# ufal/neuralmonkey

Measured on NVIDIA H100. Metric: train_target_tokens_per_sec, higher is better.
Workload: dtype f32 storage; tensor-core products in fp16 (vocabulary) / tf32 with fp32 accumulation

## Files before the change

include/nmb200.h:

```cpp
#ifndef NMB200_H
#define NMB200_H

#include <stdint.h>

#ifdef __cplusplus
extern "C" {
#endif

#define NM_ABI_VERSION 1

#define NM_OK 0
#define NM_E_INVALID (-1)
#define NM_E_UNSUPPORTED (-2)
#define NM_E_NO_DEVICE (-3)

#define NM_ACT_NONE 0
#define NM_ACT_TANH 1
#define NM_ACT_RELU 2
#define NM_ACT_SIGMOID 3

#define NM_GEMM_AUTO 0
#define NM_GEMM_SIMT 1
#define NM_GEMM_TC 2

// ... 98 lines not shown
int nm_xent_fwd(float* logits, int64_t unk_index, const int64_t* targets, const float* weights,
                float* lse, float* xent, int64_t* argmax, int64_t M, int64_t V,
                int64_t ldl, void* stream);
int nm_xent_bwd(const float* logits, const int64_t* targets, const float* weights,
                const float* lse, const float* scale, float* dlogits, int64_t M,
                int64_t V, int64_t ldl, void* stream);
int nm_log_softmax(const float* logits, const float* lse, float* logprobs,
                   int64_t M, int64_t V, int64_t ldl, void* stream);

int64_t nm_logits_xent_scratch(int64_t M, int64_t V);
int nm_logits_xent_fwd(const float* X, int64_t ldx, const float* W, int64_t ldw,
                       int transW, const float* b, int64_t unk_index, const int64_t* targets,
                       const float* weights, float* lse, float* xent,
                       int64_t* argmax, float* part, float* logits_out,
                       int64_t ldl, int64_t M, int64_t V, int64_t K, void* stream);
int nm_logits_xent_bwd(const float* X, int64_t ldx, const float* W, int64_t ldw,
                       int transW, const float* b, int64_t unk_index, const int64_t* targets,
                       const float* weights, const float* lse, const float* scale,
                       float* dlogits, int64_t ldd, int64_t M, int64_t V,
                       int64_t K, void* stream);

int nm_cast_f16(const float* src, int64_t ld_src, void* dst, int64_t ld_dst, int64_t rows,
                int64_t cols, const float* row_scale, int transpose, int extra_ones, void* stream);
int nm_gemm_f16(int64_t M, int64_t N, int64_t K, const void* A16, int64_t lda, const void* B16,
                int64_t ldb, float* C, int64_t ldc, const float* alpha_dev, const float* row_scale,
                float beta, int transposed, void* stream);
int nm_gemm_f16_tn(int64_t M, int64_t N, int64_t K, const void* A16, int64_t lda, const void* B16,
                   int64_t ldb, float* C, int64_t ldc, const float* alpha_dev, float beta, void* stream);
int nm_gemm_f16_tn_ctas(int64_t M, int64_t N, int64_t K, const void* A16, int64_t lda, const void* B16,
                        int64_t ldb, float* C, int64_t ldc, const float* alpha_dev, float beta, int max_ctas,
                        void* stream);
int nm_logits_xent_fwd16(const void* X16, int64_t ldx, const void* WT16, int64_t ldw, const float* b,
                         int64_t unk_index, const int64_t* targets, const float* weights, float* lse,
                         float* xent, int64_t* argmax, float* part, float* logits_out, int64_t ldl,
                         int64_t M, int64_t V, int64_t K, void* stream);
int nm_logits_xent_bwd16(const void* X16, int64_t ldx, const void* WT16, int64_t ldw, const float* b,
                         int64_t unk_index, const int64_t* targets, const float* mask, const float* lse,
                         void* dl16, int64_t ldd, int64_t M, int64_t V, int64_t K, void* stream);

int nm_beam_step(const float* logprobs, const float* logprob_sum,
                 const int32_t* lengths, const uint8_t* finished, float alpha,
                 float* scores, int64_t* word_ids, int32_t* beam_ids,
                 float* logprob_sum_out, int32_t* lengths_out,
                 uint8_t* finished_out, void* scratch, int64_t B, int64_t k,
                 int64_t V, void* stream);
int64_t nm_beam_scratch(int64_t B, int64_t k, int64_t V);
// ... 172 lines not shown
```

neuralmonkey_b200/build.py:

```python
import concurrent.futures
import os
import shutil
import subprocess
import sys
from typing import List

PKG_DIR = os.path.dirname(os.path.abspath(__file__))
CSRC = os.path.join(PKG_DIR, "csrc")
OBJ_DIR = os.path.join(PKG_DIR, "build")
LIB_PATH = os.path.join(PKG_DIR, "libnmb200.so")
HEADER = os.path.join(os.path.dirname(PKG_DIR), "include", "nmb200.h")

NVCC_FLAGS = [
    "-gencode", "arch=compute_90a,code=sm_90a",
    "-O3", "-lineinfo", "-std=c++17",
    "-Xcompiler", "-fPIC",
]


def _nvcc() -> str:
    nvcc = shutil.which("nvcc") or "/usr/local/cuda/bin/nvcc"
    if not os.path.exists(nvcc):
        raise RuntimeError("nvcc not found: cannot build libnmb200.so")
    return nvcc


def sources() -> List[str]:
    return sorted(f for f in os.listdir(CSRC) if f.endswith(".cu"))


def _deps_mtime() -> float:
    deps = [HEADER] + [os.path.join(CSRC, f) for f in os.listdir(CSRC)
                       if f.endswith((".cuh", ".h"))]
    return max(os.path.getmtime(d) for d in deps)


def _compile(src: str, force: bool) -> str:
    obj = os.path.join(OBJ_DIR, src[:-3] + ".o")
    src_path = os.path.join(CSRC, src)
    newest = max(os.path.getmtime(src_path), _deps_mtime())
    if not force and os.path.exists(obj) and os.path.getmtime(obj) >= newest:
        return obj
    cmd = [_nvcc()] + NVCC_FLAGS + ["-c", src_path, "-o", obj]
    res = subprocess.run(cmd, capture_output=True, text=True)
    if res.returncode != 0:
        raise RuntimeError("nvcc failed for {}:\n{}\n{}".format(
            src, res.stdout, res.stderr))
    return obj


def build(force: bool = False, verbose: bool = False) -> str:
    os.makedirs(OBJ_DIR, exist_ok=True)
    srcs = sources()
    with concurrent.futures.ThreadPoolExecutor(max_workers=8) as pool:
        objs = list(pool.map(lambda s: _compile(s, force), srcs))
    need_link = (force or not os.path.exists(LIB_PATH)
                 or any(os.path.getmtime(o) > os.path.getmtime(LIB_PATH)
                        for o in objs))
    if need_link:
        tmp_path = LIB_PATH + ".tmp.{}".format(os.getpid())
        cmd = [_nvcc(), "-shared", "-o", tmp_path] + objs + [
            "-gencode", "arch=compute_90a,code=sm_90a", "-cudart", "static"]
        res = subprocess.run(cmd, capture_output=True, text=True)
        if res.returncode != 0:
            if os.path.exists(tmp_path):
                os.remove(tmp_path)
            raise RuntimeError("link failed:\n{}\n{}".format(
                res.stdout, res.stderr))
        os.replace(tmp_path, LIB_PATH)
        if verbose:
            print("linked", LIB_PATH)
    return LIB_PATH


if __name__ == "__main__":
    print(build(force="--force" in sys.argv, verbose=True))
```

neuralmonkey_b200/csrc/gemm16.cu:

```cuda
#include <cuda_fp16.h>

#include "common.cuh"
#include "gemm_tc.h"
#include "tc_ptx.cuh"
#include "wgmma.cuh"

namespace nm {

constexpr int G16_BM = 128;
constexpr int G16_BN = 320;
constexpr int G16_A_BYTES = G16_BM * 128;
constexpr int G16_B_BYTES = G16_BN * 128;
constexpr int G16_STAGE_BYTES = G16_A_BYTES + G16_B_BYTES;
constexpr int G16_STAGES = 4;
constexpr int G16_BAR_OFF = G16_STAGES * G16_STAGE_BYTES;
constexpr int G16_SMEM_BYTES = 1024  + G16_BAR_OFF + 256 ;
constexpr int G16_THREADS = 384;
static_assert(G16_SMEM_BYTES <= 227 * 1024, "more shared memory than an sm_90 block may have");

struct G16Args {
  float* C;
  int64_t ldc;
  const float* alpha;
  const float* row_scale;
  int R, Cn, K;
  int trans_out;
  int beta;
  int vec2;
// ... 62 lines not shown
    }
    asm volatile("fence.mbarrier_init.release.cluster;" ::: "memory");
    asm volatile("fence.proxy.async.shared::cta;" ::: "memory");
  }
  __syncthreads();
  const int warp = threadIdx.x >> 5, lane = threadIdx.x & 31;

  if (warp < 4) {
    asm volatile("setmaxnreg.dec.sync.aligned.u32 40;" ::: "memory");
    if (threadIdx.x != 0) return;
    uint64_t stream_pol, keep_pol;
    asm volatile("createpolicy.fractional.L2::evict_first.b64 %0, 1.0;" : "=l"(stream_pol));
    asm volatile("createpolicy.fractional.L2::evict_last.b64 %0, 1.0;" : "=l"(keep_pol));
    int it = 0;
    for (int64_t u = begin; u < end;) {
      const int t = (int)(u / KB), kb0 = (int)(u - (int64_t)t * KB);
      const int kb1 = (int)min((int64_t)KB, end - (int64_t)t * KB);
      const int r0 = (t % tiles_r) * G16_BM, c0 = (t / tiles_r) * G16_BN;
      const int nb = min(G16_BN / 64, (p.Cn - c0 + 63) / 64);
      const int na = MN ? min(G16_BM / 64, (p.R - r0 + 63) / 64) : 1;
      const uint32_t bytes = (MN ? na * 8192 : G16_A_BYTES) + nb * 8192;
      for (int kb = kb0; kb < kb1; ++kb, ++it) {
        const int s = it % G16_STAGES;
        mbar_wait(empty(s), ((it / G16_STAGES) & 1) ^ 1u);
        mbar_expect_tx(full(s), bytes);
        const uint32_t a_dst = sbase + s * G16_STAGE_BYTES, b_dst = a_dst + G16_A_BYTES;
        if (MN) {
          for (int j = 0; j < na; ++j) tma_load_2d_hint(a_dst + j * 8192, &map_a, full(s), r0 + 64 * j, kb * 64, stream_pol);
          for (int j = 0; j < nb; ++j) tma_load_2d_hint(b_dst + j * 8192, &map_b, full(s), c0 + 64 * j, kb * 64, keep_pol);
        } else {
          tma_load_2d_hint(a_dst, &map_a, full(s), kb * 64, r0, stream_pol);
          for (int j = 0; j < nb; ++j) tma_load_2d_hint(b_dst + j * 8192, &map_b, full(s), kb * 64, c0 + 64 * j, keep_pol);
        }
      }
      u = (int64_t)t * KB + kb1;
    }
    return;
  }

  asm volatile("setmaxnreg.inc.sync.aligned.u32 232;" ::: "memory");
  const int wg = (warp >> 2) - 1, w = warp & 3, q = lane & 3;
  const float alpha = p.alpha ? __ldg(p.alpha) : 1.f;
  constexpr int KSTEP = MN ? 2048 : 32;
  float acc[128], acc2[32];
  int it = 0;
  for (int64_t u = begin; u < end;) {
    const int t = (int)(u / KB), kb0 = (int)(u - (int64_t)t * KB);
    const int kb1 = (int)min((int64_t)KB, end - (int64_t)t * KB);
    const int r0 = (t % tiles_r) * G16_BM, c0 = (t / tiles_r) * G16_BN;
#pragma unroll
    for (int i = 0; i < 128; ++i) acc[i] = 0.f;
#pragma unroll
    for (int i = 0; i < 32; ++i) acc2[i] = 0.f;
    for (int kb = kb0; kb < kb1; ++kb, ++it) {
      const int s = it % G16_STAGES;
// ... 122 lines not shown
```

neuralmonkey_b200/csrc/xent16.cu:

```cuda
#include <cuda_fp16.h>

#include "common.cuh"
#include "gemm_tc.h"
#include "tc_ptx.cuh"
#include "wgmma.cuh"

namespace nm {

__global__ void cast_f16_kernel(const float* __restrict__ src, int64_t ld_src, __half* __restrict__ dst,
                                int64_t ld_dst, int64_t rows, int64_t cols,
                                const float* __restrict__ row_scale, int extra_ones) {
  const int64_t total = rows * ld_dst;
  for (int64_t i = blockIdx.x * (int64_t)blockDim.x + threadIdx.x; i < total;
       i += (int64_t)gridDim.x * blockDim.x) {
    const int64_t r = i / ld_dst, c = i - r * ld_dst;
    float v = 0.f;
    const float sc = row_scale ? row_scale[r] : 1.f;
    if (c < cols) v = src[r * ld_src + c] * sc;
    else if (c < cols + extra_ones) v = sc;
    dst[i] = __float2half_rn(v);
  }
}

__global__ void cast_transpose_f16_kernel(const float* __restrict__ src, int64_t ld_src,
                                          __half* __restrict__ dst, int64_t ld_dst, int64_t rows,
                                          int64_t cols, const float* __restrict__ row_scale,
                                          int extra_ones) {
  __shared__ float tile[32][33];
  const int64_t r0 = blockIdx.x * 32LL, c0 = blockIdx.y * 32LL;
  for (int i = threadIdx.y; i < 32; i += blockDim.y) {
    const int64_t r = r0 + i, c = c0 + threadIdx.x;
    float v = 0.f;
    if (r < rows) {
      const float sc = row_scale ? row_scale[r] : 1.f;
      if (c < cols) v = src[r * ld_src + c] * sc;
      else if (c < cols + extra_ones) v = sc;
    }
    tile[i][threadIdx.x] = v;
  }
  __syncthreads();
  for (int i = threadIdx.y; i < 32; i += blockDim.y) {
    const int64_t c = c0 + i, r = r0 + threadIdx.x;
    if (c < cols + extra_ones && r < ld_dst) dst[c * ld_dst + r] = __float2half_rn(tile[threadIdx.x][i]);
  }
}

constexpr int X16_BM = 64;
constexpr int X16_BN = TC_XENT_BN;
constexpr int X16_A_BYTES = X16_BM * 128;
constexpr int X16_B_BYTES = X16_BN * 128;
constexpr int X16_B_SLOTS = XENT16_MAX_K / 64;
constexpr int X16_STAGE_WARP = 16 * 128 * 2;
constexpr int X16_THREADS = 384;

template <bool BWD>
struct X16Cfg {
  static constexpr int A_STAGES = BWD ? 4 : 8;
  static constexpr int A_OFF = X16_B_SLOTS * X16_B_BYTES;
  static constexpr int ST_OFF = A_OFF + A_STAGES * X16_A_BYTES;
// ... 53 lines not shown
  const int first = (int)((int64_t)blockIdx.x * units / gridDim.x);
  const int count = (int)((int64_t)(blockIdx.x + 1) * units / gridDim.x) - first;
  const int KB = (p.K + 63) / 64;

  if (threadIdx.x == 0) {
    asm volatile("prefetch.tensormap [%0];" ::"l"(reinterpret_cast<uint64_t>(&map_x)) : "memory");
    asm volatile("prefetch.tensormap [%0];" ::"l"(reinterpret_cast<uint64_t>(&map_w)) : "memory");
    for (int s = 0; s < AST; ++s) {
      mbar_init(full_a(s), 1);
      mbar_init(empty_a(s), 4);
    }
    for (int s = 0; s < X16_B_SLOTS; ++s) {
      mbar_init(full_b(s), 1);
      mbar_init(empty_b(s), 4);
    }
    asm volatile("fence.mbarrier_init.release.cluster;" ::: "memory");
    asm volatile("fence.proxy.async.shared::cta;" ::: "memory");
  }
  __syncthreads();
  const int warp = threadIdx.x >> 5, lane = threadIdx.x & 31;

  if (warp < 4) {
    asm volatile("setmaxnreg.dec.sync.aligned.u32 40;" ::: "memory");
    if (threadIdx.x != 0) return;
    int loads = 0, prev_tn = -1;
    for (int j = 0; j < count; ++j) {
      const int u = first + j, tm = u % tiles_m, tn = u / tiles_m;
      const bool reload = tn != prev_tn;
      loads += reload;
      prev_tn = tn;
      for (int kb = 0; kb < KB; ++kb) {
        const int ia = j * KB + kb, sa = ia % AST;
        mbar_wait(empty_a(sa), ((ia / AST) & 1) ^ 1u);
        mbar_expect_tx(full_a(sa), X16_A_BYTES);
        tma_load_2d(sbase + Cfg::A_OFF + sa * X16_A_BYTES, &map_x, full_a(sa), kb * 64, tm * X16_BM);
        if (reload) {
          mbar_wait(empty_b(kb), ((loads - 1) & 1) ^ 1u);
          mbar_expect_tx(full_b(kb), X16_B_BYTES);
          tma_load_2d(sbase + kb * X16_B_BYTES, &map_w, full_b(kb), kb * 64, tn * X16_BN);
        }
      }
    }
    return;
  }

  asm volatile("setmaxnreg.inc.sync.aligned.u32 232;" ::: "memory");
  const int c = (warp >> 2) - 1;
  const int w = warp & 3, q = lane & 3;
  uint64_t evict_first = 0;
  if (BWD) asm volatile("createpolicy.fractional.L2::evict_first.b64 %0, 1.0;" : "=l"(evict_first));
  if (c == 1) named_arrive(1);
  float acc[128];
  int loads = 0, prev_tn = -1;
  for (int j = 0; j < count; ++j) {
    const int u = first + j, tm = u % tiles_m, tn = u / tiles_m;
    loads += tn != prev_tn;
    prev_tn = tn;
    if ((j & 1) != c) continue;
    const bool last_use = j + 1 == count || (u + 1) / tiles_m != tn;

    named_sync(1 + c);
#pragma unroll
    for (int i = 0; i < 128; ++i) acc[i] = 0.f;
    for (int kb = 0; kb < KB; ++kb) {
      const int ia = j * KB + kb, sa = ia % AST;
      mbar_wait(full_a(sa), (ia / AST) & 1);
      mbar_wait(full_b(kb), (loads - 1) & 1);
      const uint32_t a_addr = sbase + Cfg::A_OFF + sa * X16_A_BYTES, b_addr = sbase + kb * X16_B_BYTES;
      wgmma_fence();
#pragma unroll
      for (int k = 0; k < 4; ++k)
        Wgmma<256, 2>::mma(acc, gmma_desc_sw128(a_addr + k * 32), gmma_desc_sw128(b_addr + k * 32));
      wgmma_commit();
      wgmma_wait<1>();
      wgmma_fence_operands(acc);
      if (kb > 0 && lane == 0) mbar_arrive(empty_a((ia - 1) % AST));
    }
    wgmma_wait<0>();
    wgmma_fence_operands(acc);
    if (lane == 0) {
      mbar_arrive(empty_a((j * KB + KB - 1) % AST));
      if (last_use)
        for (int kb = 0; kb < KB; ++kb) mbar_arrive(empty_b(kb));
    }
    if (j + 1 < count) named_arrive(2 - c);

    const int r0 = tm * X16_BM + 16 * w + (lane >> 2);
    const int n0 = tn * X16_BN, cb = n0 + 2 * q;
    const int V = p.V;
#pragma unroll
    for (int i = 0; i < 32; ++i) {
#pragma unroll
      for (int e = 0; e < 2; ++e) {
        const int col = cb + 8 * i + e;
        const float b = (p.bias != nullptr && col < V) ? __ldg(p.bias + col) : 0.f;
        acc[4 * i + e] += b;
        acc[4 * i + 2 + e] += b;
      }
    }
    const int unk_rel = (int)(p.unk - cb);
    if (p.unk >= 0 && unk_rel >= 0 && unk_rel < X16_BN && (unk_rel & 6) == 0) {
#pragma unroll
      for (int i = 0; i < 32; ++i)
#pragma unroll
        for (int e = 0; e < 2; ++e)
          if (8 * i + e == unk_rel) {
            acc[4 * i + e] += -1e9f;
            acc[4 * i + 2 + e] += -1e9f;
          }
    }
#pragma unroll
    for (int h = 0; h < 2; ++h) {
      const int row = r0 + 8 * h;
      const bool row_ok = row < p.M;
      const int target = (row_ok && p.targets) ? (int)p.targets[row] : -1;
      const int t_rel = target - cb;
      const bool has_t = target >= 0 && t_rel >= 0 && t_rel < X16_BN && (t_rel & 6) == 0;
      if constexpr (!BWD) {
        if (p.logits && row_ok) {
          float* lrow = p.logits + (int64_t)row * p.ldl + cb;
          const int ncols = V - cb;
#pragma unroll
          for (int i = 0; i < 32; ++i)
#pragma unroll
            for (int e = 0; e < 2; ++e)
              if (8 * i + e < ncols) lrow[8 * i + e] = acc[4 * i + 2 * h + e];
        }
        if (n0 + X16_BN > V) {
#pragma unroll
          for (int i = 0; i < 32; ++i)
#pragma unroll
            for (int e = 0; e < 2; ++e)
              if (cb + 8 * i + e >= V) acc[4 * i + 2 * h + e] = -INFINITY;
        }
        float mx = -INFINITY;
        int arg = 0x7fffffff;
#pragma unroll
        for (int i = 0; i < 32; ++i)
#pragma unroll
          for (int e = 0; e < 2; ++e)
            if (acc[4 * i + 2 * h + e] > mx) {
              mx = acc[4 * i + 2 * h + e];
              arg = cb + 8 * i + e;
            }
        const float m2 = mx == -INFINITY ? 0.f : mx * TC_LOG2E;
        float s[4] = {0.f, 0.f, 0.f, 0.f};
#pragma unroll
        for (int i = 0; i < 32; ++i)
#pragma unroll
          for (int e = 0; e < 2; ++e)
            s[(2 * i + e) & 3] += fast_ex2(fmaf(acc[4 * i + 2 * h + e], TC_LOG2E, -m2));
        float sum = (s[0] + s[1]) + (s[2] + s[3]);
        float tgt = -INFINITY;
        if (has_t) {
#pragma unroll
          for (int i = 0; i < 32; ++i)
#pragma unroll
            for (int e = 0; e < 2; ++e)
              if (8 * i + e == t_rel) tgt = acc[4 * i + 2 * h + e];
        }
        merge_stats(mx, sum, arg, tgt, __shfl_xor_sync(0xffffffffu, mx, 1), __shfl_xor_sync(0xffffffffu, sum, 1),
                    __shfl_xor_sync(0xffffffffu, arg, 1), __shfl_xor_sync(0xffffffffu, tgt, 1));
        if (row_ok && (q & 1) == h) {
          const int tiles_n2 = 2 * ((V + X16_BN - 1) / X16_BN);
          p.part[(int64_t)row * tiles_n2 + 2 * tn + (q >> 1)] = make_float4(mx, sum, __int_as_float(arg), tgt);
        }
      } else {
        const float lse2 = row_ok ? p.lse[row] * TC_LOG2E : 0.f;
        const float wt = row_ok ? (p.mask ? p.mask[row] : 1.f) : 0.f;
#pragma unroll
        for (int i = 0; i < 32; ++i)
#pragma unroll
          for (int e = 0; e < 2; ++e)
            acc[4 * i + 2 * h + e] = fast_ex2(fmaf(acc[4 * i + 2 * h + e], TC_LOG2E, -lse2)) * wt;
        if (has_t) {
#pragma unroll
          for (int i = 0; i < 32; ++i)
#pragma unroll
            for (int e = 0; e < 2; ++e)
              if (8 * i + e == t_rel) acc[4 * i + 2 * h + e] -= wt;
        }
      }
    }
    if constexpr (BWD) {
      uint8_t* stage = smem + Cfg::ST_OFF + (warp - 4) * X16_STAGE_WARP;
      const uint32_t stage_u = smem_u32(stage);
      const int srow_w = (lane & 7) + ((lane >> 3) & 1) * 8;
#pragma unroll
      for (int half = 0; half < 2; ++half) {
#pragma unroll
        for (int jj = 0; jj < 16; jj += 2) {
          const int i = 16 * half + jj;
          const int chunk = jj + (lane >> 4);
          const uint32_t addr = stage_u + srow_w * 256 + ((chunk ^ (srow_w & 7)) << 4);
          asm volatile("stmatrix.sync.aligned.m8n8.x4.shared.b16 [%0], {%1, %2, %3, %4};" ::"r"(addr),
                       "r"(pack_half2(acc[4 * i], acc[4 * i + 1])), "r"(pack_half2(acc[4 * i + 2], acc[4 * i + 3])),
                       "r"(pack_half2(acc[4 * i + 4], acc[4 * i + 5])), "r"(pack_half2(acc[4 * i + 6], acc[4 * i + 7]))
                       : "memory");
        }
        __syncwarp();
#pragma unroll
        for (int it = 0; it < 8; ++it) {
          const int idx = it * 32 + lane, srow = idx >> 4, ch = idx & 15;
          const uint4 v = *reinterpret_cast<const uint4*>(stage + srow * 256 + ((ch ^ (srow & 7)) << 4));
          const int grow = tm * X16_BM + 16 * w + srow;
          const int gcol = n0 + 128 * half + 8 * ch;
          if (grow < p.M && gcol < V) {
            __half* dst = p.dl16 + (int64_t)grow * p.ldd + gcol;
            if (gcol + 8 <= V) {
              asm volatile("st.global.L2::cache_hint.v4.b32 [%0], {%1, %2, %3, %4}, %5;" ::"l"(dst), "r"(v.x),
                           "r"(v.y), "r"(v.z), "r"(v.w), "l"(evict_first)
                           : "memory");
            } else {
              const uint32_t wv[4] = {v.x, v.y, v.z, v.w};
#pragma unroll
              for (int e = 0; e < 8; ++e)
                if (gcol + e < V) dst[e] = __ushort_as_half((unsigned short)(wv[e >> 1] >> (16 * (e & 1))));
            }
          }
        }
        __syncwarp();
      }
    }
  }
}

template <bool BWD>
static int launch_xent16(const CUtensorMap& mx, const CUtensorMap& mw, const X16Args& a, int grid, cudaStream_t s,
                         const char* name) {
  auto kern = xent16_kernel<BWD>;
  static bool attr_done = false;
  if (!attr_done) {
    NM_CUDA_TRY(cudaFuncSetAttribute(kern, cudaFuncAttributeMaxDynamicSharedMemorySize, X16Cfg<BWD>::SMEM_BYTES));
    attr_done = true;
  }
  kern<<<grid, X16_THREADS, X16Cfg<BWD>::SMEM_BYTES, s>>>(mx, mw, a);
  NM_LAUNCH_CHECK(name);
  return NM_OK;
}

int xent16_launch(bool bwd, const void* X16, int64_t ldx, const void* WT16, int64_t ldw, const float* b,
                  int64_t unk_index, const int64_t* targets, const float* mask, const float* lse, float4* part,
                  float* logits_out, int64_t ldl, void* dl16, int64_t ldd, int64_t M, int64_t V, int64_t K,
                  cudaStream_t s) {
// ... 10 lines not shown
  int rc = make_map16(&mx, X16, M, K, ldx, X16_BM);
  if (rc) return rc;
  rc = make_map16(&mw, WT16, V, K, ldw, X16_BN);
  if (rc) return rc;
  X16Args a{b, unk_index, targets, mask, lse, part, logits_out, ldl, reinterpret_cast<__half*>(dl16), ldd,
            (int)M, (int)V, (int)K};
  const int64_t units = ceil_div(M, X16_BM) * ceil_div(V, X16_BN);
  const int grid = (int)(units < sm_count() ? units : sm_count());
  return bwd ? launch_xent16<true>(mx, mw, a, grid, s, name) : launch_xent16<false>(mx, mw, a, grid, s, name);
}

}

using namespace nm;

extern "C" {

int nm_cast_f16(const float* src, int64_t ld_src, void* dst, int64_t ld_dst, int64_t rows, int64_t cols,
                const float* row_scale, int transpose, int extra_ones, void* stream) {
  NM_REQUIRE(src && dst && rows > 0 && cols > 0 && ld_src >= cols, NM_E_INVALID, "nm_cast_f16: bad arguments");
  cudaStream_t s = (cudaStream_t)stream;
  if (!transpose) {
    NM_REQUIRE(extra_ones >= 0 && ld_dst >= cols + extra_ones, NM_E_INVALID, "nm_cast_f16: bad destination pitch");
    const int64_t total = rows * ld_dst;
    const int64_t blocks = ceil_div(total, 256 * 4);
    const int64_t cap = (int64_t)sm_count() * 16;
    cast_f16_kernel<<<(unsigned)(blocks < cap ? blocks : cap), 256, 0, s>>>(
        src, ld_src, reinterpret_cast<__half*>(dst), ld_dst, rows, cols, row_scale, extra_ones);
  } else {
    NM_REQUIRE(ld_dst >= rows && extra_ones >= 0, NM_E_INVALID, "nm_cast_f16: bad destination pitch");
    const dim3 grid((unsigned)ceil_div(ld_dst, 32), (unsigned)ceil_div(cols + extra_ones, 32));
    cast_transpose_f16_kernel<<<grid, dim3(32, 8), 0, s>>>(src, ld_src, reinterpret_cast<__half*>(dst), ld_dst,
                                                          rows, cols, row_scale, extra_ones);
  }
  NM_LAUNCH_CHECK("nm_cast_f16");
  return NM_OK;
}

int nm_logits_xent_bwd16(const void* X16, int64_t ldx, const void* WT16, int64_t ldw, const float* b,
                         int64_t unk_index, const int64_t* targets, const float* mask, const float* lse,
                         void* dl16, int64_t ldd, int64_t M, int64_t V, int64_t K, void* stream) {
  NM_REQUIRE(X16 && WT16 && targets && lse && dl16, NM_E_INVALID, "nm_logits_xent_bwd16: null pointer");
  NM_REQUIRE(M > 0 && V > 0 && K > 0 && ldx >= K && ldw >= K && ldd >= V, NM_E_INVALID,
             "nm_logits_xent_bwd16: bad sizes");
  if (K <= XENT16_MAX_K)
    return xent16_launch(true, X16, ldx, WT16, ldw, b, unk_index, targets, mask, lse, nullptr, nullptr, 0, dl16,
                         ldd, M, V, K, (cudaStream_t)stream);
  TcEpilogue epi{};
  epi.mode = TC_EPI_XENT_BWD16;
  epi.bias = b;
  epi.unk_index = unk_index;
  epi.targets = targets;
  epi.weights = mask;
  epi.lse = lse;
  TcExt ext{};
  ext.C16 = dl16;
  ext.ldc16 = ldd;
  return tc_gemm16_launch(M, V, K, X16, ldx, WT16, ldw, epi, ext, (cudaStream_t)stream);
// ... 4 lines not shown
```

neuralmonkey_b200/lib.py:

```python
import ctypes
import os
from typing import Dict, Optional, Sequence

import torch

_PKG_DIR = os.path.dirname(os.path.abspath(__file__))
LIB_PATH = os.path.join(_PKG_DIR, "libnmb200.so")

NM_ACT = {None: 0, "none": 0, "tanh": 1, "relu": 2, "sigmoid": 3}
GEMM_AUTO, GEMM_SIMT, GEMM_TC = 0, 1, 2

HEADER_PATH = os.path.join(os.path.dirname(_PKG_DIR), "include", "nmb200.h")


def parse_header(path: str = HEADER_PATH) -> Dict[str, str]:
    import re
    text = open(path, encoding="utf-8").read()
    text = re.sub(r"/\*.*?\*/", " ", text, flags=re.S)
    text = re.sub(r"^\s*#.*$", " ", text, flags=re.M)
    sigs = {}
    for m in re.finditer(r"(const char\*|int64_t|int)\s+(nm_\w+)\s*\(([^)]*)\)\s*;", text):
        ret, name, args = m.group(1), m.group(2), m.group(3).strip()
        codes = ""
        if args and args != "void":
# ... 15 lines not shown
        sigs[name] = (rcode, codes)
    return sigs


_CTYPES = {"p": ctypes.c_void_p, "i": ctypes.c_int, "l": ctypes.c_int64,
           "f": ctypes.c_float, "d": ctypes.c_double}


class NMB200Error(RuntimeError):
    """A libnmb200 call returned a non-zero status."""


_lib = None


def load() -> ctypes.CDLL:
    global _lib
    if _lib is not None:
        return _lib
    if not os.path.exists(LIB_PATH):
        raise NMB200Error(
            "libnmb200.so not found at {}: run `python -m neuralmonkey_b200.build` "
            "(there is no CPU fallback)".format(LIB_PATH))
    lib = ctypes.CDLL(LIB_PATH)
    restypes = {"s": ctypes.c_char_p, "l": ctypes.c_int64, "i": ctypes.c_int}
    for name, (rcode, codes) in parse_header().items():
        fn = getattr(lib, name)
        fn.restype = restypes[rcode]
        fn.argtypes = [_CTYPES[c] for c in codes]
    _lib = lib
    return lib


def declared_symbols() -> Sequence[str]:
    return sorted(parse_header())


def _stream() -> int:
    return torch.cuda.current_stream().cuda_stream


def ptr(t: Optional[torch.Tensor]) -> Optional[int]:
    if t is None:
        return None
    if not t.is_cuda:
        raise NMB200Error("libnmb200 got a non-CUDA tensor: there is no CPU path")
    return t.data_ptr()


_profile = None


def profile_start() -> None:
# ... 54 lines not shown
```

neuralmonkey_b200/ops.py:

```python
from typing import Optional, Sequence, Tuple

import ctypes

import torch

from neuralmonkey_b200 import lib
from neuralmonkey_b200.lib import call, ptr

_GEMM_BACKEND = lib.GEMM_AUTO


def set_gemm_backend(name: str) -> None:
    global _GEMM_BACKEND
    _GEMM_BACKEND = {"auto": lib.GEMM_AUTO, "simt": lib.GEMM_SIMT, "tc": lib.GEMM_TC}[name]


def gemm_backend() -> int:
    return _GEMM_BACKEND


def _f32(t: torch.Tensor) -> torch.Tensor:
    if t.dtype != torch.float32:
        raise TypeError("expected float32, got {}".format(t.dtype))
    return t
# ... 664 lines not shown
        dw = w_sink if w_sink is not None else torch.zeros(w_shape, device=x.device, dtype=torch.float32)
        if trans_w:
            dw.index_add_(0, targets, gx)
            dw.sub_((gx.sum(0) / vocab).unsqueeze(0))
        else:
            dw.index_add_(1, targets, gx.t().contiguous())
            dw.sub_((gx.sum(0) / vocab).unsqueeze(1))
        db = None
        if has_bias:
            db = b_sink if b_sink is not None else torch.zeros(vocab, device=x.device, dtype=torch.float32)
            db.index_add_(0, targets, g)
            db.sub_(g.sum() / vocab)
        return (dx, None if w_sink is not None else dw, None if (b_sink is not None or not has_bias) else db,
                None, None, None)


def smoothing_term(x: torch.Tensor, w: torch.Tensor, b: Optional[torch.Tensor], targets: torch.Tensor,
                   unk_index: int = -1, trans_w: bool = False) -> torch.Tensor:
    return _SmoothingTerm.apply(x, w, b, targets, unk_index, trans_w)


_DW16_CTAS = 48


def _pad8(n: int) -> int:
    return (n + 7) // 8 * 8


class _LogitsXent16(torch.autograd.Function):

    @staticmethod
    def forward(ctx, x, w, b, targets, weights, unk_index, keep_logits):
        x2 = x.reshape(-1, x.shape[-1])
        x2, ldx = _rows(x2)
        m, k = x2.shape
        v = w.size(1)
        dev = x.device
        kpad = _pad8(k)
        targets = targets.reshape(-1).contiguous()
        weights = weights.reshape(-1).contiguous()
        w2, ldw = _rows(w)
        x16 = torch.empty(m, kpad, device=dev, dtype=torch.float16)
        call("nm_cast_f16", ptr(x2), ldx, ptr(x16), kpad, m, k, None, 0, 0, lib.stream())
        wt16 = torch.empty(v, kpad, device=dev, dtype=torch.float16)
        call("nm_cast_f16", ptr(w2), ldw, ptr(wt16), kpad, k, v, None, 1, 0, lib.stream())
        lse = torch.empty(m, device=dev, dtype=torch.float32)
        xent = torch.empty(m, device=dev, dtype=torch.float32)
        argmax = torch.empty(m, device=dev, dtype=torch.int64)
        logits = torch.empty(m, v, device=dev, dtype=torch.float32) if keep_logits else None
        part = torch.empty(lib.load().nm_logits_xent_scratch(m, v), device=dev, dtype=torch.float32)
        call("nm_logits_xent_fwd16", ptr(x16), kpad, ptr(wt16), kpad, ptr(b), unk_index, ptr(targets),
             ptr(weights), ptr(lse), ptr(xent), ptr(argmax), ptr(part), ptr(logits), v, m, v, k,
             lib.stream())
        ctx.save_for_backward(x2, w2, b, targets, weights, lse, x16, wt16)
        ctx.cfg = (unk_index, x.shape)
        ctx.sinks = (_sink(w), _sink(b) if b is not None else None)
        ctx.mark_non_differentiable(lse, argmax)
        if keep_logits:
            ctx.mark_non_differentiable(logits)
        return xent, lse, argmax, logits

    @staticmethod
    def backward(ctx, dxent, _dlse, _dargmax, _dlogits):
        x2, w2, b, targets, weights, lse, x16, wt16 = ctx.saved_tensors
        unk_index, in_shape = ctx.cfg
        m, k = x2.shape
        v = w2.size(1)
        dev = x2.device
        kpad, vpad = _pad8(k), _pad8(v)
        _, ldx = _rows(x2)
        _, ldw = _rows(w2)
        dl16 = torch.empty(m, vpad, device=dev, dtype=torch.float16)
        call("nm_logits_xent_bwd16", ptr(x16), kpad, ptr(wt16), kpad, ptr(b), unk_index, ptr(targets),
             ptr(weights), ptr(lse), ptr(dl16), vpad, m, v, k, lib.stream())
        upstream = dxent.reshape(-1).to(torch.float32).contiguous()
        dx = None
        if ctx.needs_input_grad[0]:
            w16 = torch.empty(k, vpad, device=dev, dtype=torch.float16)
            call("nm_cast_f16", ptr(w2), ldw, ptr(w16), vpad, k, v, None, 0, 0, lib.stream())
            dx = torch.empty(m, k, device=dev, dtype=torch.float32)
            call("nm_gemm_f16", m, k, v, ptr(dl16), vpad, ptr(w16), vpad, ptr(dx), k, None,
                 ptr(upstream), 0.0, 0, lib.stream())
            dx = dx.view(in_shape)
        w_sink, _b_sink = ctx.sinks
        smax = upstream.abs().amax().clamp_min(1e-30).reshape(1)
        k1pad = _pad8(k + 1)
        xs16 = torch.empty(m, k1pad, device=dev, dtype=torch.float16)
        call("nm_cast_f16", ptr(x2), ldx, ptr(xs16), k1pad, m, k, ptr(upstream / smax), 0, 1, lib.stream())
        sink_aug = torch.as_strided(w_sink, (k + 1, v), (v, 1))

        def dw():
            args = (k + 1, v, m, ptr(xs16), k1pad, ptr(dl16), vpad, ptr(sink_aug), v, ptr(smax), 1.0)
            if _wg["open"]:
                call("nm_gemm_f16_tn_ctas", *args, _DW16_CTAS, lib.stream())
            else:
                call("nm_gemm_f16_tn", *args, lib.stream())
        _off_the_chain(dw, xs16, dl16, smax, sink_aug)
# ... 792 lines not shown
```

Measured before the change: 1.310 million.

## Fold vocabulary bias into fp16 GEMM via augmented ones columns and vectorize casts

The bias is appended to the transposed fp16 weight as two extra K rows, a hi part and an fp16 rounding residual, and two ones columns are appended to the fp16 activations. The logits GEMM then produces biased logits directly, and the per-element bias loads in the xent epilogues are skipped. The cast kernel is vectorized to write eight halves per thread, and the fwd/bwd epilogues are restructured: target/lse loads are hoisted before the GEMM and the max/argmax/sum reductions are split into independent passes. The change also adds compile-time probe modes, left off by default, plus a variant-build helper; the extra K columns may add a k-block when K crosses a multiple of 64.

Result: faster. 1.339 million, median of 6 (+2.3%).

```diff
diff --git a/include/nmb200.h b/include/nmb200.h
--- a/include/nmb200.h
+++ b/include/nmb200.h
@@ -144,6 +144,8 @@
 
 int nm_cast_f16(const float* src, int64_t ld_src, void* dst, int64_t ld_dst, int64_t rows,
                 int64_t cols, const float* row_scale, int transpose, int extra_ones, void* stream);
+int nm_cast_f16_wt(const float* W, int64_t ldw, const float* b, void* WT16, int64_t ldt, int64_t K,
+                   int64_t V, void* stream);
 int nm_gemm_f16(int64_t M, int64_t N, int64_t K, const void* A16, int64_t lda, const void* B16,
                 int64_t ldb, float* C, int64_t ldc, const float* alpha_dev, const float* row_scale,
                 float beta, int transposed, void* stream);
diff --git a/neuralmonkey_b200/build.py b/neuralmonkey_b200/build.py
--- a/neuralmonkey_b200/build.py
+++ b/neuralmonkey_b200/build.py
@@ -3,7 +3,7 @@
 import shutil
 import subprocess
 import sys
-from typing import List
+from typing import List, Sequence
 
 PKG_DIR = os.path.dirname(os.path.abspath(__file__))
 CSRC = os.path.join(PKG_DIR, "csrc")
@@ -35,13 +35,13 @@
     return max(os.path.getmtime(d) for d in deps)
 
 
-def _compile(src: str, force: bool) -> str:
-    obj = os.path.join(OBJ_DIR, src[:-3] + ".o")
+def _compile(src: str, force: bool, obj_dir: str = OBJ_DIR, defines: Sequence[str] = ()) -> str:
+    obj = os.path.join(obj_dir, src[:-3] + ".o")
     src_path = os.path.join(CSRC, src)
     newest = max(os.path.getmtime(src_path), _deps_mtime())
     if not force and os.path.exists(obj) and os.path.getmtime(obj) >= newest:
         return obj
-    cmd = [_nvcc()] + NVCC_FLAGS + ["-c", src_path, "-o", obj]
+    cmd = [_nvcc()] + NVCC_FLAGS + ["-D" + d for d in defines] + ["-c", src_path, "-o", obj]
     res = subprocess.run(cmd, capture_output=True, text=True)
     if res.returncode != 0:
         raise RuntimeError("nvcc failed for {}:\n{}\n{}".format(
@@ -54,23 +54,37 @@
     srcs = sources()
     with concurrent.futures.ThreadPoolExecutor(max_workers=8) as pool:
         objs = list(pool.map(lambda s: _compile(s, force), srcs))
-    need_link = (force or not os.path.exists(LIB_PATH)
-                 or any(os.path.getmtime(o) > os.path.getmtime(LIB_PATH)
-                        for o in objs))
-    if need_link:
-        tmp_path = LIB_PATH + ".tmp.{}".format(os.getpid())
-        cmd = [_nvcc(), "-shared", "-o", tmp_path] + objs + [
-            "-gencode", "arch=compute_90a,code=sm_90a", "-cudart", "static"]
-        res = subprocess.run(cmd, capture_output=True, text=True)
-        if res.returncode != 0:
-            if os.path.exists(tmp_path):
-                os.remove(tmp_path)
-            raise RuntimeError("link failed:\n{}\n{}".format(
-                res.stdout, res.stderr))
-        os.replace(tmp_path, LIB_PATH)
-        if verbose:
-            print("linked", LIB_PATH)
+    if _link(objs, LIB_PATH, force) and verbose:
+        print("linked", LIB_PATH)
     return LIB_PATH
+
+
+def _link(objs: List[str], path: str, force: bool) -> bool:
+    if not (force or not os.path.exists(path)
+            or any(os.path.getmtime(o) > os.path.getmtime(path) for o in objs)):
+        return False
+    tmp_path = path + ".tmp.{}".format(os.getpid())
+    cmd = [_nvcc(), "-shared", "-o", tmp_path] + objs + [
+        "-gencode", "arch=compute_90a,code=sm_90a", "-cudart", "static"]
+    res = subprocess.run(cmd, capture_output=True, text=True)
+    if res.returncode != 0:
+        if os.path.exists(tmp_path):
+            os.remove(tmp_path)
+        raise RuntimeError("link failed:\n{}\n{}".format(
+            res.stdout, res.stderr))
+    os.replace(tmp_path, path)
+    return True
+
+
+def build_variant(src: str, define: str, out_dir: str) -> str:
+    build()
+    obj_dir = os.path.join(out_dir, "obj_" + define.replace("=", "_"))
+    os.makedirs(obj_dir, exist_ok=True)
+    objs = [_compile(s, False, obj_dir, [define]) if s == src else os.path.join(OBJ_DIR, s[:-3] + ".o")
+            for s in sources()]
+    path = os.path.join(out_dir, "libnmb200_{}.so".format(define.replace("=", "_")))
+    _link(objs, path, False)
+    return path
 
 
 if __name__ == "__main__":
diff --git a/neuralmonkey_b200/csrc/gemm16.cu b/neuralmonkey_b200/csrc/gemm16.cu
--- a/neuralmonkey_b200/csrc/gemm16.cu
+++ b/neuralmonkey_b200/csrc/gemm16.cu
@@ -4,6 +4,10 @@
 #include "gemm_tc.h"
 #include "tc_ptx.cuh"
 #include "wgmma.cuh"
+
+#ifndef NM_GEMM16_PROBE
+#define NM_GEMM16_PROBE 0
+#endif
 
 namespace nm {
 
@@ -112,15 +116,16 @@
       const uint32_t bytes = (MN ? na * 8192 : G16_A_BYTES) + nb * 8192;
       for (int kb = kb0; kb < kb1; ++kb, ++it) {
         const int s = it % G16_STAGES;
+        const int nbl = NM_GEMM16_PROBE == 1 && it >= G16_STAGES ? 0 : nb;
         mbar_wait(empty(s), ((it / G16_STAGES) & 1) ^ 1u);
-        mbar_expect_tx(full(s), bytes);
+        mbar_expect_tx(full(s), bytes - (nb - nbl) * 8192);
         const uint32_t a_dst = sbase + s * G16_STAGE_BYTES, b_dst = a_dst + G16_A_BYTES;
         if (MN) {
           for (int j = 0; j < na; ++j) tma_load_2d_hint(a_dst + j * 8192, &map_a, full(s), r0 + 64 * j, kb * 64, stream_pol);
-          for (int j = 0; j < nb; ++j) tma_load_2d_hint(b_dst + j * 8192, &map_b, full(s), c0 + 64 * j, kb * 64, keep_pol);
+          for (int j = 0; j < nbl; ++j) tma_load_2d_hint(b_dst + j * 8192, &map_b, full(s), c0 + 64 * j, kb * 64, keep_pol);
         } else {
           tma_load_2d_hint(a_dst, &map_a, full(s), kb * 64, r0, stream_pol);
-          for (int j = 0; j < nb; ++j) tma_load_2d_hint(b_dst + j * 8192, &map_b, full(s), kb * 64, c0 + 64 * j, keep_pol);
+          for (int j = 0; j < nbl; ++j) tma_load_2d_hint(b_dst + j * 8192, &map_b, full(s), kb * 64, c0 + 64 * j, keep_pol);
         }
       }
       u = (int64_t)t * KB + kb1;
diff --git a/neuralmonkey_b200/csrc/xent16.cu b/neuralmonkey_b200/csrc/xent16.cu
--- a/neuralmonkey_b200/csrc/xent16.cu
+++ b/neuralmonkey_b200/csrc/xent16.cu
@@ -5,27 +5,47 @@
 #include "tc_ptx.cuh"
 #include "wgmma.cuh"
 
+#ifndef NM_XENT16_PROBE
+#define NM_XENT16_PROBE 0
+#endif
+
 namespace nm {
 
 __global__ void cast_f16_kernel(const float* __restrict__ src, int64_t ld_src, __half* __restrict__ dst,
                                 int64_t ld_dst, int64_t rows, int64_t cols,
-                                const float* __restrict__ row_scale, int extra_ones) {
-  const int64_t total = rows * ld_dst;
+                                const float* __restrict__ row_scale, int extra_ones, int vec) {
+  const int64_t chunks = (ld_dst + 7) >> 3, total = rows * chunks;
   for (int64_t i = blockIdx.x * (int64_t)blockDim.x + threadIdx.x; i < total;
        i += (int64_t)gridDim.x * blockDim.x) {
-    const int64_t r = i / ld_dst, c = i - r * ld_dst;
-    float v = 0.f;
+    const int64_t r = i / chunks, c0 = (i - r * chunks) << 3;
     const float sc = row_scale ? row_scale[r] : 1.f;
-    if (c < cols) v = src[r * ld_src + c] * sc;
-    else if (c < cols + extra_ones) v = sc;
-    dst[i] = __float2half_rn(v);
+    const float* s = src + r * ld_src;
+    __half2 h[4];
+#pragma unroll
+    for (int e = 0; e < 8; e += 2) {
+      float v[2];
+#pragma unroll
+      for (int k = 0; k < 2; ++k) {
+        const int64_t c = c0 + e + k;
+        v[k] = c < cols ? s[c] * sc : (c < cols + extra_ones ? sc : 0.f);
+      }
+      h[e >> 1] = __floats2half2_rn(v[0], v[1]);
+    }
+    __half* d = dst + r * ld_dst + c0;
+    if (vec) {
+      *reinterpret_cast<uint4*>(d) = *reinterpret_cast<const uint4*>(h);
+    } else {
+#pragma unroll
+      for (int e = 0; e < 8; ++e)
+        if (c0 + e < ld_dst) d[e] = e & 1 ? __high2half(h[e >> 1]) : __low2half(h[e >> 1]);
+    }
   }
 }
 
 __global__ void cast_transpose_f16_kernel(const float* __restrict__ src, int64_t ld_src,
                                           __half* __restrict__ dst, int64_t ld_dst, int64_t rows,
                                           int64_t cols, const float* __restrict__ row_scale,
-                                          int extra_ones) {
+                                          int extra_ones, const float* __restrict__ bias) {
   __shared__ float tile[32][33];
   const int64_t r0 = blockIdx.x * 32LL, c0 = blockIdx.y * 32LL;
   for (int i = threadIdx.y; i < 32; i += blockDim.y) {
@@ -35,6 +55,9 @@
       const float sc = row_scale ? row_scale[r] : 1.f;
       if (c < cols) v = src[r * ld_src + c] * sc;
       else if (c < cols + extra_ones) v = sc;
+    } else if (bias != nullptr && r < rows + 2 && c < cols) {
+      const float b = bias[c];
+      v = r == rows ? b : b - __half2float(__float2half_rn(b));
     }
     tile[i][threadIdx.x] = v;
   }
@@ -134,7 +157,7 @@
 
   if (warp < 4) {
     asm volatile("setmaxnreg.dec.sync.aligned.u32 40;" ::: "memory");
-    if (threadIdx.x != 0) return;
+    if (threadIdx.x != 0 || NM_XENT16_PROBE == 2) return;
     int loads = 0, prev_tn = -1;
     for (int j = 0; j < count; ++j) {
       const int u = first + j, tm = u % tiles_m, tn = u / tiles_m;
@@ -144,8 +167,12 @@
       for (int kb = 0; kb < KB; ++kb) {
         const int ia = j * KB + kb, sa = ia % AST;
         mbar_wait(empty_a(sa), ((ia / AST) & 1) ^ 1u);
-        mbar_expect_tx(full_a(sa), X16_A_BYTES);
-        tma_load_2d(sbase + Cfg::A_OFF + sa * X16_A_BYTES, &map_x, full_a(sa), kb * 64, tm * X16_BM);
+        if (NM_XENT16_PROBE == 3 && ia >= AST) {
+          mbar_arrive(full_a(sa));
+        } else {
+          mbar_expect_tx(full_a(sa), X16_A_BYTES);
+          tma_load_2d(sbase + Cfg::A_OFF + sa * X16_A_BYTES, &map_x, full_a(sa), kb * 64, tm * X16_BM);
+        }
         if (reload) {
           mbar_wait(empty_b(kb), ((loads - 1) & 1) ^ 1u);
           mbar_expect_tx(full_b(kb), X16_B_BYTES);
@@ -170,11 +197,24 @@
     prev_tn = tn;
     if ((j & 1) != c) continue;
     const bool last_use = j + 1 == count || (u + 1) / tiles_m != tn;
+    const int r0 = tm * X16_BM + 16 * w + (lane >> 2);
+    int target[2];
+    float lse2[2], wt[2];
+#pragma unroll
+    for (int h = 0; h < 2; ++h) {
+      const int row = r0 + 8 * h;
+      const bool row_ok = row < p.M;
+      target[h] = (row_ok && p.targets) ? (int)p.targets[row] : -1;
+      if (BWD) {
+        lse2[h] = row_ok ? p.lse[row] * TC_LOG2E : 0.f;
+        wt[h] = row_ok ? (p.mask ? p.mask[row] : 1.f) : 0.f;
+      }
+    }
 
     named_sync(1 + c);
 #pragma unroll
-    for (int i = 0; i < 128; ++i) acc[i] = 0.f;
-    for (int kb = 0; kb < KB; ++kb) {
+    for (int i = 0; i < 128; ++i) acc[i] = NM_XENT16_PROBE == 2 ? (float)((i * 37 + lane + j) & 63) * 0.125f : 0.f;
+    for (int kb = 0; kb < (NM_XENT16_PROBE == 2 ? 0 : KB); ++kb) {
       const int ia = j * KB + kb, sa = ia % AST;
       mbar_wait(full_a(sa), (ia / AST) & 1);
       mbar_wait(full_b(kb), (loads - 1) & 1);
@@ -196,18 +236,26 @@
         for (int kb = 0; kb < KB; ++kb) mbar_arrive(empty_b(kb));
     }
     if (j + 1 < count) named_arrive(2 - c);
-
-    const int r0 = tm * X16_BM + 16 * w + (lane >> 2);
+    if (NM_XENT16_PROBE == 1) {
+      uint32_t bits = 0;
+#pragma unroll
+      for (int i = 0; i < 128; ++i) bits |= __float_as_uint(acc[i]);
+      if (bits == 0x7fc00001u && p.part) p.part[0] = make_float4(0.f, 0.f, 0.f, 0.f);
+      continue;
+    }
+
     const int n0 = tn * X16_BN, cb = n0 + 2 * q;
     const int V = p.V;
-#pragma unroll
-    for (int i = 0; i < 32; ++i) {
-#pragma unroll
-      for (int e = 0; e < 2; ++e) {
-        const int col = cb + 8 * i + e;
-        const float b = (p.bias != nullptr && col < V) ? __ldg(p.bias + col) : 0.f;
-        acc[4 * i + e] += b;
-        acc[4 * i + 2 + e] += b;
+    if (p.bias != nullptr) {
+#pragma unroll
+      for (int i = 0; i < 32; ++i) {
+#pragma unroll
+        for (int e = 0; e < 2; ++e) {
+          const int col = cb + 8 * i + e;
+          const float b = col < V ? __ldg(p.bias + col) : 0.f;
+          acc[4 * i + e] += b;
+          acc[4 * i + 2 + e] += b;
+        }
       }
     }
     const int unk_rel = (int)(p.unk - cb);
@@ -221,15 +269,19 @@
             acc[4 * i + 2 + e] += -1e9f;
           }
     }
+    int t_rel[2];
+    bool has_t[2];
 #pragma unroll
     for (int h = 0; h < 2; ++h) {
-      const int row = r0 + 8 * h;
-      const bool row_ok = row < p.M;
-      const int target = (row_ok && p.targets) ? (int)p.targets[row] : -1;
-      const int t_rel = target - cb;
-      const bool has_t = target >= 0 && t_rel >= 0 && t_rel < X16_BN && (t_rel & 6) == 0;
-      if constexpr (!BWD) {
-        if (p.logits && row_ok) {
+      t_rel[h] = target[h] - cb;
+      has_t[h] = target[h] >= 0 && t_rel[h] >= 0 && t_rel[h] < X16_BN && (t_rel[h] & 6) == 0;
+    }
+    if constexpr (!BWD) {
+      if (p.logits) {
+#pragma unroll
+        for (int h = 0; h < 2; ++h) {
+          const int row = r0 + 8 * h;
+          if (row >= p.M) continue;
           float* lrow = p.logits + (int64_t)row * p.ldl + cb;
           const int ncols = V - cb;
 #pragma unroll
@@ -238,63 +290,83 @@
             for (int e = 0; e < 2; ++e)
               if (8 * i + e < ncols) lrow[8 * i + e] = acc[4 * i + 2 * h + e];
         }
-        if (n0 + X16_BN > V) {
+      }
+      if (n0 + X16_BN > V) {
+#pragma unroll
+        for (int i = 0; i < 32; ++i)
+#pragma unroll
+          for (int e = 0; e < 2; ++e)
+            if (cb + 8 * i + e >= V) acc[4 * i + e] = acc[4 * i + 2 + e] = -INFINITY;
+      }
+      auto row_max = [&](int h) {
+        float mk[4] = {-INFINITY, -INFINITY, -INFINITY, -INFINITY};
+#pragma unroll
+        for (int i = 0; i < 32; ++i)
+#pragma unroll
+          for (int e = 0; e < 2; ++e) mk[(2 * i + e) & 3] = fmaxf(mk[(2 * i + e) & 3], acc[4 * i + 2 * h + e]);
+        return fmaxf(fmaxf(mk[0], mk[1]), fmaxf(mk[2], mk[3]));
+      };
+      auto row_arg = [&](int h, float mx) {
+        int argk[4] = {X16_BN, X16_BN, X16_BN, X16_BN};
+#pragma unroll
+        for (int i = 31; i >= 0; --i)
+#pragma unroll
+          for (int e = 1; e >= 0; --e)
+            if (acc[4 * i + 2 * h + e] == mx) argk[(2 * i + e) & 3] = 8 * i + e;
+        const int a = min(min(argk[0], argk[1]), min(argk[2], argk[3]));
+        return mx == -INFINITY ? 0x7fffffff : cb + a;
+      };
+      auto row_sum = [&](int h, float mx) {
+        const float m2 = mx == -INFINITY ? 0.f : mx * TC_LOG2E;
+        float sk[4] = {0.f, 0.f, 0.f, 0.f};
+#pragma unroll
+        for (int i = 0; i < 32; ++i)
+#pragma unroll
+          for (int e = 0; e < 2; ++e) sk[(2 * i + e) & 3] += fast_ex2(fmaf(acc[4 * i + 2 * h + e], TC_LOG2E, -m2));
+        return (sk[0] + sk[1]) + (sk[2] + sk[3]);
+      };
+      auto row_tgt = [&](int h) {
+        float tgt = -INFINITY;
+        if (has_t[h]) {
 #pragma unroll
           for (int i = 0; i < 32; ++i)
 #pragma unroll
             for (int e = 0; e < 2; ++e)
-              if (cb + 8 * i + e >= V) acc[4 * i + 2 * h + e] = -INFINITY;
-        }
-        float mx = -INFINITY;
-        int arg = 0x7fffffff;
-#pragma unroll
-        for (int i = 0; i < 32; ++i)
-#pragma unroll
-          for (int e = 0; e < 2; ++e)
-            if (acc[4 * i + 2 * h + e] > mx) {
-              mx = acc[4 * i + 2 * h + e];
-              arg = cb + 8 * i + e;
-            }
-        const float m2 = mx == -INFINITY ? 0.f : mx * TC_LOG2E;
-        float s[4] = {0.f, 0.f, 0.f, 0.f};
-#pragma unroll
-        for (int i = 0; i < 32; ++i)
-#pragma unroll
-          for (int e = 0; e < 2; ++e)
-            s[(2 * i + e) & 3] += fast_ex2(fmaf(acc[4 * i + 2 * h + e], TC_LOG2E, -m2));
-        float sum = (s[0] + s[1]) + (s[2] + s[3]);
-        float tgt = -INFINITY;
-        if (has_t) {
+              if (8 * i + e == t_rel[h]) tgt = acc[4 * i + 2 * h + e];
+        }
+        return tgt;
+      };
+      float mx0 = row_max(0), mx1 = row_max(1);
+      int arg0 = row_arg(0, mx0), arg1 = row_arg(1, mx1);
+      float sum0 = row_sum(0, mx0), sum1 = row_sum(1, mx1);
+      float tgt0 = row_tgt(0), tgt1 = row_tgt(1);
+      merge_stats(mx0, sum0, arg0, tgt0, __shfl_xor_sync(0xffffffffu, mx0, 1), __shfl_xor_sync(0xffffffffu, sum0, 1),
+                  __shfl_xor_sync(0xffffffffu, arg0, 1), __shfl_xor_sync(0xffffffffu, tgt0, 1));
+      merge_stats(mx1, sum1, arg1, tgt1, __shfl_xor_sync(0xffffffffu, mx1, 1), __shfl_xor_sync(0xffffffffu, sum1, 1),
+                  __shfl_xor_sync(0xffffffffu, arg1, 1), __shfl_xor_sync(0xffffffffu, tgt1, 1));
+      const bool odd = (q & 1) != 0;
+      const int row = r0 + (odd ? 8 : 0);
+      if (row < p.M) {
+        const int tiles_n2 = 2 * ((V + X16_BN - 1) / X16_BN);
+        p.part[(int64_t)row * tiles_n2 + 2 * tn + (q >> 1)] =
+            odd ? make_float4(mx1, sum1, __int_as_float(arg1), tgt1) : make_float4(mx0, sum0, __int_as_float(arg0), tgt0);
+      }
+    } else {
+#pragma unroll
+      for (int i = 0; i < 32; ++i)
+#pragma unroll
+        for (int k = 0; k < 4; ++k)
+          acc[4 * i + k] = fast_ex2(fmaf(acc[4 * i + k], TC_LOG2E, -lse2[k >> 1])) * wt[k >> 1];
+#pragma unroll
+      for (int h = 0; h < 2; ++h) {
+        if (has_t[h]) {
 #pragma unroll
           for (int i = 0; i < 32; ++i)
 #pragma unroll
             for (int e = 0; e < 2; ++e)
-              if (8 * i + e == t_rel) tgt = acc[4 * i + 2 * h + e];
-        }
-        merge_stats(mx, sum, arg, tgt, __shfl_xor_sync(0xffffffffu, mx, 1), __shfl_xor_sync(0xffffffffu, sum, 1),
-                    __shfl_xor_sync(0xffffffffu, arg, 1), __shfl_xor_sync(0xffffffffu, tgt, 1));
-        if (row_ok && (q & 1) == h) {
-          const int tiles_n2 = 2 * ((V + X16_BN - 1) / X16_BN);
-          p.part[(int64_t)row * tiles_n2 + 2 * tn + (q >> 1)] = make_float4(mx, sum, __int_as_float(arg), tgt);
-        }
-      } else {
-        const float lse2 = row_ok ? p.lse[row] * TC_LOG2E : 0.f;
-        const float wt = row_ok ? (p.mask ? p.mask[row] : 1.f) : 0.f;
-#pragma unroll
-        for (int i = 0; i < 32; ++i)
-#pragma unroll
-          for (int e = 0; e < 2; ++e)
-            acc[4 * i + 2 * h + e] = fast_ex2(fmaf(acc[4 * i + 2 * h + e], TC_LOG2E, -lse2)) * wt;
-        if (has_t) {
-#pragma unroll
-          for (int i = 0; i < 32; ++i)
-#pragma unroll
-            for (int e = 0; e < 2; ++e)
-              if (8 * i + e == t_rel) acc[4 * i + 2 * h + e] -= wt;
-        }
-      }
-    }
-    if constexpr (BWD) {
+              if (8 * i + e == t_rel[h]) acc[4 * i + 2 * h + e] -= wt[h];
+        }
+      }
       uint8_t* stage = smem + Cfg::ST_OFF + (warp - 4) * X16_STAGE_WARP;
       const uint32_t stage_u = smem_u32(stage);
       const int srow_w = (lane & 7) + ((lane >> 3) & 1) * 8;
@@ -311,27 +383,32 @@
                        : "memory");
         }
         __syncwarp();
+        uint4 v[8];
 #pragma unroll
         for (int it = 0; it < 8; ++it) {
           const int idx = it * 32 + lane, srow = idx >> 4, ch = idx & 15;
-          const uint4 v = *reinterpret_cast<const uint4*>(stage + srow * 256 + ((ch ^ (srow & 7)) << 4));
+          v[it] = *reinterpret_cast<const uint4*>(stage + srow * 256 + ((ch ^ (srow & 7)) << 4));
+        }
+        __syncwarp();
+#pragma unroll
+        for (int it = 0; it < 8; ++it) {
+          const int idx = it * 32 + lane, srow = idx >> 4, ch = idx & 15;
           const int grow = tm * X16_BM + 16 * w + srow;
           const int gcol = n0 + 128 * half + 8 * ch;
           if (grow < p.M && gcol < V) {
             __half* dst = p.dl16 + (int64_t)grow * p.ldd + gcol;
             if (gcol + 8 <= V) {
-              asm volatile("st.global.L2::cache_hint.v4.b32 [%0], {%1, %2, %3, %4}, %5;" ::"l"(dst), "r"(v.x),
-                           "r"(v.y), "r"(v.z), "r"(v.w), "l"(evict_first)
+              asm volatile("st.global.L2::cache_hint.v4.b32 [%0], {%1, %2, %3, %4}, %5;" ::"l"(dst), "r"(v[it].x),
+                           "r"(v[it].y), "r"(v[it].z), "r"(v[it].w), "l"(evict_first)
                            : "memory");
             } else {
-              const uint32_t wv[4] = {v.x, v.y, v.z, v.w};
+              const uint32_t wv[4] = {v[it].x, v[it].y, v[it].z, v[it].w};
 #pragma unroll
               for (int e = 0; e < 8; ++e)
                 if (gcol + e < V) dst[e] = __ushort_as_half((unsigned short)(wv[e >> 1] >> (16 * (e & 1))));
             }
           }
         }
-        __syncwarp();
       }
     }
   }
@@ -388,18 +465,30 @@
   cudaStream_t s = (cudaStream_t)stream;
   if (!transpose) {
     NM_REQUIRE(extra_ones >= 0 && ld_dst >= cols + extra_ones, NM_E_INVALID, "nm_cast_f16: bad destination pitch");
-    const int64_t total = rows * ld_dst;
-    const int64_t blocks = ceil_div(total, 256 * 4);
+    const int64_t total = rows * ceil_div(ld_dst, 8);
+    const int64_t blocks = ceil_div(total, 256);
     const int64_t cap = (int64_t)sm_count() * 16;
+    const int vec = (ld_dst & 7) == 0 && (reinterpret_cast<uintptr_t>(dst) & 15) == 0;
     cast_f16_kernel<<<(unsigned)(blocks < cap ? blocks : cap), 256, 0, s>>>(
-        src, ld_src, reinterpret_cast<__half*>(dst), ld_dst, rows, cols, row_scale, extra_ones);
+        src, ld_src, reinterpret_cast<__half*>(dst), ld_dst, rows, cols, row_scale, extra_ones, vec);
   } else {
     NM_REQUIRE(ld_dst >= rows && extra_ones >= 0, NM_E_INVALID, "nm_cast_f16: bad destination pitch");
     const dim3 grid((unsigned)ceil_div(ld_dst, 32), (unsigned)ceil_div(cols + extra_ones, 32));
     cast_transpose_f16_kernel<<<grid, dim3(32, 8), 0, s>>>(src, ld_src, reinterpret_cast<__half*>(dst), ld_dst,
-                                                          rows, cols, row_scale, extra_ones);
+                                                          rows, cols, row_scale, extra_ones, nullptr);
   }
   NM_LAUNCH_CHECK("nm_cast_f16");
+  return NM_OK;
+}
+
+int nm_cast_f16_wt(const float* W, int64_t ldw, const float* b, void* WT16, int64_t ldt, int64_t K, int64_t V,
+                   void* stream) {
+  NM_REQUIRE(W && b && WT16 && K > 0 && V > 0 && ldw >= V && ldt >= K + 2, NM_E_INVALID,
+             "nm_cast_f16_wt: bad arguments");
+  const dim3 grid((unsigned)ceil_div(ldt, 32), (unsigned)ceil_div(V, 32));
+  cast_transpose_f16_kernel<<<grid, dim3(32, 8), 0, (cudaStream_t)stream>>>(
+      W, ldw, reinterpret_cast<__half*>(WT16), ldt, K, V, nullptr, 0, b);
+  NM_LAUNCH_CHECK("nm_cast_f16_wt");
   return NM_OK;
 }
 
diff --git a/neuralmonkey_b200/lib.py b/neuralmonkey_b200/lib.py
--- a/neuralmonkey_b200/lib.py
+++ b/neuralmonkey_b200/lib.py
@@ -61,13 +61,17 @@
         raise NMB200Error(
             "libnmb200.so not found at {}: run `python -m neuralmonkey_b200.build` "
             "(there is no CPU fallback)".format(LIB_PATH))
-    lib = ctypes.CDLL(LIB_PATH)
+    _lib = load_from(LIB_PATH)
+    return _lib
+
+
+def load_from(path: str) -> ctypes.CDLL:
+    lib = ctypes.CDLL(path)
     restypes = {"s": ctypes.c_char_p, "l": ctypes.c_int64, "i": ctypes.c_int}
     for name, (rcode, codes) in parse_header().items():
         fn = getattr(lib, name)
         fn.restype = restypes[rcode]
         fn.argtypes = [_CTYPES[c] for c in codes]
-    _lib = lib
     return lib
 
 
diff --git a/neuralmonkey_b200/ops.py b/neuralmonkey_b200/ops.py
--- a/neuralmonkey_b200/ops.py
+++ b/neuralmonkey_b200/ops.py
@@ -710,6 +710,8 @@
 
 _DW16_CTAS = 48
 
+_XENT16_MAX_K = 320
+
 
 def _pad8(n: int) -> int:
     return (n + 7) // 8 * 8
@@ -724,24 +726,29 @@
         m, k = x2.shape
         v = w.size(1)
         dev = x.device
-        kpad = _pad8(k)
         targets = targets.reshape(-1).contiguous()
         weights = weights.reshape(-1).contiguous()
         w2, ldw = _rows(w)
+        kx = k + 2 if k + 2 <= _XENT16_MAX_K else k
+        kpad = _pad8(kx)
         x16 = torch.empty(m, kpad, device=dev, dtype=torch.float16)
-        call("nm_cast_f16", ptr(x2), ldx, ptr(x16), kpad, m, k, None, 0, 0, lib.stream())
+        call("nm_cast_f16", ptr(x2), ldx, ptr(x16), kpad, m, k, None, 0, kx - k, lib.stream())
         wt16 = torch.empty(v, kpad, device=dev, dtype=torch.float16)
-        call("nm_cast_f16", ptr(w2), ldw, ptr(wt16), kpad, k, v, None, 1, 0, lib.stream())
+        if kx > k:
+            call("nm_cast_f16_wt", ptr(w2), ldw, ptr(b), ptr(wt16), kpad, k, v, lib.stream())
+        else:
+            call("nm_cast_f16", ptr(w2), ldw, ptr(wt16), kpad, k, v, None, 1, 0, lib.stream())
+        b16 = None if kx > k else b
         lse = torch.empty(m, device=dev, dtype=torch.float32)
         xent = torch.empty(m, device=dev, dtype=torch.float32)
         argmax = torch.empty(m, device=dev, dtype=torch.int64)
         logits = torch.empty(m, v, device=dev, dtype=torch.float32) if keep_logits else None
         part = torch.empty(lib.load().nm_logits_xent_scratch(m, v), device=dev, dtype=torch.float32)
-        call("nm_logits_xent_fwd16", ptr(x16), kpad, ptr(wt16), kpad, ptr(b), unk_index, ptr(targets),
-             ptr(weights), ptr(lse), ptr(xent), ptr(argmax), ptr(part), ptr(logits), v, m, v, k,
+        call("nm_logits_xent_fwd16", ptr(x16), kpad, ptr(wt16), kpad, ptr(b16), unk_index, ptr(targets),
+             ptr(weights), ptr(lse), ptr(xent), ptr(argmax), ptr(part), ptr(logits), v, m, v, kx,
              lib.stream())
-        ctx.save_for_backward(x2, w2, b, targets, weights, lse, x16, wt16)
-        ctx.cfg = (unk_index, x.shape)
+        ctx.save_for_backward(x2, w2, b16, targets, weights, lse, x16, wt16)
+        ctx.cfg = (unk_index, x.shape, kx)
         ctx.sinks = (_sink(w), _sink(b) if b is not None else None)
         ctx.mark_non_differentiable(lse, argmax)
         if keep_logits:
@@ -750,17 +757,17 @@
 
     @staticmethod
     def backward(ctx, dxent, _dlse, _dargmax, _dlogits):
-        x2, w2, b, targets, weights, lse, x16, wt16 = ctx.saved_tensors
-        unk_index, in_shape = ctx.cfg
+        x2, w2, b16, targets, weights, lse, x16, wt16 = ctx.saved_tensors
+        unk_index, in_shape, kx = ctx.cfg
         m, k = x2.shape
         v = w2.size(1)
         dev = x2.device
-        kpad, vpad = _pad8(k), _pad8(v)
+        kpad, vpad = _pad8(kx), _pad8(v)
         _, ldx = _rows(x2)
         _, ldw = _rows(w2)
         dl16 = torch.empty(m, vpad, device=dev, dtype=torch.float16)
-        call("nm_logits_xent_bwd16", ptr(x16), kpad, ptr(wt16), kpad, ptr(b), unk_index, ptr(targets),
-             ptr(weights), ptr(lse), ptr(dl16), vpad, m, v, k, lib.stream())
+        call("nm_logits_xent_bwd16", ptr(x16), kpad, ptr(wt16), kpad, ptr(b16), unk_index, ptr(targets),
+             ptr(weights), ptr(lse), ptr(dl16), vpad, m, v, kx, lib.stream())
         upstream = dxent.reshape(-1).to(torch.float32).contiguous()
         dx = None
         if ctx.needs_input_grad[0]:
```
